# LarsDoorenbos/ccdm-stochastic-segmentation

Measured on AMD Instinct MI355X. Metric: segmentation samples/sec, LIDC 128x128 T=250, higher is better.
Workload: dtype f32 (conv products as split fp16 hi/lo x3 on MFMA, fp32 accumulate)

## Files before the change

ccdm_stochastic_segmentation_amd/csrc/ccdm_engine.hip:

```cpp
#include "ccdm_common.h"

#include <map>
#include <vector>

namespace ccdm {

__global__ void k_step_set(int32_t* p, int32_t v) { *p = v; }
__global__ void k_step_inc(int32_t* p) { *p += 1; }
__global__ void k_run_set(ccdm_post_run* dst, const ccdm_post_run v) { *dst = v; }
__global__ __launch_bounds__(256) void k_absmax(const float* __restrict__ x, size_t n4, float* out) {
    float m = 0.f;
    bool bad = false;
    for (size_t i = (size_t)blockIdx.x * blockDim.x + threadIdx.x; i < n4; i += (size_t)gridDim.x * blockDim.x) {
        const float4 v = reinterpret_cast<const float4*>(x)[i];
        bad |= !(fabsf(v.x) <= 3.0e38f) | !(fabsf(v.y) <= 3.0e38f) | !(fabsf(v.z) <= 3.0e38f) | !(fabsf(v.w) <= 3.0e38f);
        m = fmaxf(m, fmaxf(fmaxf(fabsf(v.x), fabsf(v.y)), fmaxf(fabsf(v.z), fabsf(v.w))));
    }
    if (bad) m = __builtin_inff();
#pragma unroll
    for (int off = 32; off > 0; off >>= 1) m = fmaxf(m, __shfl_xor(m, off));
    if ((threadIdx.x & 63) == 0) atomicMax(reinterpret_cast<unsigned*>(out), __float_as_uint(m));
}

struct Op {
    int kind;
    ccdm_conv_args conv;
    const float* qkv; float* out; int N, T, C, heads, order;
    const double* fin; double* fout; int S_in, S_out;
    ccdm_attn_block_args ab;
    ccdm_resample_args rs;
    ccdm_stem_args st;
    ccdm_head_args hd;
};

static int launch_op(const Op& op, hipStream_t s) {
    switch (op.kind) {
        case 6: return fail("engine: the head + epilogue op is launched with the epilogue's arguments");
        case 0: return launch_conv(op.conv, s);
        case 1: return launch_attention(op.qkv, op.out, op.N, op.T, op.T, op.C, op.heads, op.order, s);
        case 2: return launch_stats_fold(op.fin, op.N, op.S_in, op.C, op.S_out, op.fout, s);
        case 3: return launch_attn_block(op.ab, s);
        case 4: return launch_resample(op.rs, s);
        default: return launch_stem(op.st, s);
    }
}

}

struct ccdm_engine {
    int32_t* step = nullptr;
    std::vector<ccdm::Op> ops;
    ccdm_post_args post{};
    bool has_post = false;
    ccdm_post_run run{};
    ccdm_post_run* run_dev = nullptr;
    bool run_dirty = false;
    int next_row = 0;
    hipGraph_t graph = nullptr;
    hipGraphExec_t exec = nullptr;
    bool graph_valid = false;
    int graph_with_epilogue = -1;
    int captures = 0;
    struct Tap { std::vector<hipEvent_t> ev; int n = 0; };
    std::map<int, Tap> taps;
};

using namespace ccdm;

static void drop_graph(ccdm_engine* e) {
    if (e->exec) { (void)hipGraphExecDestroy(e->exec); e->exec = nullptr; }
    if (e->graph) { (void)hipGraphDestroy(e->graph); e->graph = nullptr; }
    e->graph_valid = false;
}

static int launch_step(ccdm_engine* e, int with_epilogue, hipStream_t s, bool profile) {
    for (size_t i = 0; i < e->ops.size(); ++i) {
        const Op& op = e->ops[i];
        ccdm_engine::Tap* tp = nullptr;
        if (profile) {
            auto it = e->taps.find((int)i);
            if (it != e->taps.end() && (size_t)(2 * it->second.n + 1) < it->second.ev.size()) tp = &it->second;
        }
        if (tp) (void)hipEventRecord(tp->ev[2 * tp->n], s);
        int rc;
        if (op.kind == 6) {
            rc = (with_epilogue && e->has_post) ? launch_head(op.hd, e->post, s) : fail("engine_run: this step ends in a fused head + epilogue op: with_epilogue must be 1 and an epilogue set");
        } else rc = launch_op(op, s);
        if (tp) { (void)hipEventRecord(tp->ev[2 * tp->n + 1], s); tp->n++; }
        if (rc) return rc;
    }
    if (with_epilogue && e->has_post && !(e->ops.size() && e->ops.back().kind == 6)) {
        int rc = launch_posterior(e->post, s);
        if (rc) return rc;
    }
    hipLaunchKernelGGL(k_step_inc, dim3(1), dim3(1), 0, s, e->step);
    CCDM_CHECK_LAUNCH("step_inc");
    return 0;
}

extern "C" ccdm_engine* ccdm_engine_create(int32_t* step_counter) {
    if (!step_counter) { fail("engine_create: null step counter"); return nullptr; }
    ccdm_engine* e = new ccdm_engine();
    e->step = step_counter;
    return e;
}

extern "C" void ccdm_engine_destroy(ccdm_engine* e) {
    if (!e) return;
    drop_graph(e);
    for (auto& kv : e->taps)
        for (hipEvent_t ev : kv.second.ev) (void)hipEventDestroy(ev);
    delete e;
}

extern "C" int ccdm_engine_add_conv(ccdm_engine* e, const ccdm_conv_args* a) {
    CCDM_REQUIRE(e && a, "engine_add_conv: null");
    Op op{};
    op.kind = 0;
    op.conv = *a;
    op.conv.step_ptr = e->step;
    e->ops.push_back(op);
    drop_graph(e);
    return (int)e->ops.size() - 1;
}

extern "C" int ccdm_engine_add_attention(ccdm_engine* e, const float* qkv, float* out, int N, int T, int C, int heads, int order) {
    CCDM_REQUIRE(e && qkv && out, "engine_add_attention: null");
    Op op{};
    op.kind = 1;
// ... 38 lines not shown
    CCDM_REQUIRE(e && a, "engine_add_stem: null");
    CCDM_REQUIRE(ccdm_stem_conv_supported(a->Cs, a->Cout, a->H, a->W, CCDM_PREC_F16X3), "engine_add_stem: Cs=%d Cout=%d %dx%d is not built", a->Cs, a->Cout, a->H, a->W);
    Op op{};
    op.kind = 5;
    op.st = *a;
    e->ops.push_back(op);
    drop_graph(e);
    return (int)e->ops.size() - 1;
}

extern "C" int ccdm_engine_add_head_posterior(ccdm_engine* e, const ccdm_head_args* a) {
    CCDM_REQUIRE(e && a, "engine_add_head_posterior: null");
    CCDM_REQUIRE(ccdm_head_posterior_supported(a->C, a->K, a->H, a->W, CCDM_PREC_F16X3), "engine_add_head_posterior: C=%d K=%d %dx%d is not built", a->C, a->K, a->H, a->W);
    Op op{};
    op.kind = 6;
    op.hd = *a;
    e->ops.push_back(op);
    drop_graph(e);
    return (int)e->ops.size() - 1;
}

extern "C" int ccdm_engine_set_epilogue(ccdm_engine* e, const ccdm_post_args* a) {
    CCDM_REQUIRE(e && a, "engine_set_epilogue: null");
    e->post = *a;
    e->post.step_ptr = e->step;
    e->has_post = true;
    if (e->run_dev) {
        e->post.run = e->run_dev;
        const ccdm_post_args& p = e->post;
        e->run = ccdm_post_run{p.noise, p.noise_step_stride, p.philox_seed, p.sample_offset, p.noise_row0, p.out_probs, p.out_onehot, p.posterior_out};
        e->run_dirty = true;
    }
    drop_graph(e);
    return 0;
}

extern "C" int ccdm_engine_num_ops(const ccdm_engine* e) { return e ? (int)e->ops.size() : -1; }
extern "C" int ccdm_engine_num_captures(const ccdm_engine* e) { return e ? e->captures : -1; }

extern "C" int ccdm_engine_set_run_block(ccdm_engine* e, void* dev_block) {
    CCDM_REQUIRE(e && e->has_post, "engine_set_run_block: no epilogue set");
    CCDM_REQUIRE(dev_block && (reinterpret_cast<uintptr_t>(dev_block) & 7) == 0, "engine_set_run_block: null or misaligned block");
    e->run_dev = static_cast<ccdm_post_run*>(dev_block);
    e->post.run = e->run_dev;
    const ccdm_post_args& p = e->post;
    e->run = ccdm_post_run{p.noise, p.noise_step_stride, p.philox_seed, p.sample_offset, p.noise_row0, p.out_probs, p.out_onehot, p.posterior_out};
    e->run_dirty = true;
    drop_graph(e);
    return 0;
}

extern "C" int ccdm_engine_set_run(ccdm_engine* e, const float* noise, int64_t noise_step_stride, int32_t noise_row0, uint64_t philox_seed,
                                   uint32_t sample_offset, float* out_probs, int64_t* out_onehot, float* posterior_out) {
    CCDM_REQUIRE(e && e->has_post, "engine_set_run: no epilogue set");
    if (e->run_dev) {
        const ccdm_post_run r{noise, noise_step_stride, philox_seed, sample_offset, noise_row0, out_probs, out_onehot, posterior_out};
        const ccdm_post_run& o = e->run;
        const bool same = o.noise == r.noise && o.noise_step_stride == r.noise_step_stride && o.philox_seed == r.philox_seed &&
                          o.sample_offset == r.sample_offset && o.noise_row0 == r.noise_row0 && o.out_probs == r.out_probs &&
                          o.out_onehot == r.out_onehot && o.posterior_out == r.posterior_out;
        if (!same) { e->run = r; e->run_dirty = true; }
        return 0;
    }
    ccdm_post_args& p = e->post;
    const bool same = p.noise == noise && p.noise_step_stride == noise_step_stride && p.noise_row0 == noise_row0 && p.philox_seed == philox_seed &&
                      p.sample_offset == sample_offset && p.out_probs == out_probs && p.out_onehot == out_onehot &&
                      p.posterior_out == posterior_out;
    if (!same) drop_graph(e);
    p.noise = noise; p.noise_step_stride = noise_step_stride; p.noise_row0 = noise_row0; p.philox_seed = philox_seed; p.sample_offset = sample_offset;
    p.out_probs = out_probs; p.out_onehot = out_onehot; p.posterior_out = posterior_out;
    return 0;
}

extern "C" int ccdm_engine_run(ccdm_engine* e, int first_row, int n_steps, int with_epilogue, int use_graph, void* stream) {
    CCDM_REQUIRE(e, "engine_run: null engine");
    CCDM_REQUIRE(n_steps >= 0, "engine_run: n_steps=%d", n_steps);
    hipStream_t s = (hipStream_t)stream;
    hipLaunchKernelGGL(k_step_set, dim3(1), dim3(1), 0, s, e->step, (int32_t)first_row);
    CCDM_CHECK_LAUNCH("step_set");
    e->next_row = first_row + n_steps;
    if (e->run_dev && e->run_dirty) {
        hipLaunchKernelGGL(k_run_set, dim3(1), dim3(1), 0, s, e->run_dev, e->run);
        CCDM_CHECK_LAUNCH("run_set");
        e->run_dirty = false;
    }
    const bool profile = !e->taps.empty();
    if (profile) {
        use_graph = 0;
        if (first_row == 0) for (auto& kv : e->taps) kv.second.n = 0;
    }
    if (use_graph) {
        if (!e->graph_valid || e->graph_with_epilogue != with_epilogue) {
            drop_graph(e);
            hipError_t err = hipStreamBeginCapture(s, hipStreamCaptureModeRelaxed);
            if (err != hipSuccess) return fail("engine_run: BeginCapture: %s", hipGetErrorString(err));
            const int rc = launch_step(e, with_epilogue, s, false);
            err = hipStreamEndCapture(s, &e->graph);
            if (rc) { if (e->graph) { (void)hipGraphDestroy(e->graph); e->graph = nullptr; } return rc; }
            if (err != hipSuccess) return fail("engine_run: EndCapture: %s", hipGetErrorString(err));
            err = hipGraphInstantiate(&e->exec, e->graph, nullptr, nullptr, 0);
            if (err != hipSuccess) return fail("engine_run: GraphInstantiate: %s", hipGetErrorString(err));
            e->graph_valid = true;
            e->graph_with_epilogue = with_epilogue;
            e->captures++;
        }
        for (int i = 0; i < n_steps; ++i) {
            hipError_t err = hipGraphLaunch(e->exec, s);
            if (err != hipSuccess) return fail("engine_run: GraphLaunch: %s", hipGetErrorString(err));
        }
        return 0;
    }
    for (int i = 0; i < n_steps; ++i) {
        int rc = launch_step(e, with_epilogue, s, profile);
        if (rc) return rc;
    }
    return 0;
}

extern "C" int ccdm_engine_profile_op(ccdm_engine* e, int op_index, int capacity) {
    CCDM_REQUIRE(e, "engine_profile_op: null engine");
    if (op_index < 0) {
        for (auto& kv : e->taps)
            for (hipEvent_t ev : kv.second.ev) (void)hipEventDestroy(ev);
        e->taps.clear();
        return 0;
    }
    CCDM_REQUIRE(op_index < (int)e->ops.size(), "engine_profile_op: op %d out of range", op_index);
    ccdm_engine::Tap& t = e->taps[op_index];
    t.n = 0;
    while ((int)t.ev.size() < 2 * capacity) {
        hipEvent_t ev;
        if (hipEventCreate(&ev) != hipSuccess) return fail("engine_profile_op: hipEventCreate failed");
        t.ev.push_back(ev);
    }
    return 0;
}

extern "C" int ccdm_engine_profile_read(ccdm_engine* e, int op_index, double* mean_ms, double* min_ms, double* max_ms) {
    CCDM_REQUIRE(e, "engine_profile_read: null engine");
    auto it = e->taps.find(op_index);
    CCDM_REQUIRE(it != e->taps.end(), "engine_profile_read: op %d is not tapped", op_index);
    ccdm_engine::Tap& t = it->second;
    double sum = 0, mn = 1e30, mx = 0;
    int n = 0;
    for (int i = 0; i < t.n; ++i) {
        float ms = 0.f;
// ... 67 lines not shown
```

ccdm_stochastic_segmentation_amd/engine.py:

```python
from __future__ import annotations

import ctypes as C
import math
from dataclasses import dataclass
from typing import Dict, List, Optional, Sequence, Tuple

import numpy as np
import torch

from . import hip
from .unet_spec import GN_EPS, UNetSpec


@dataclass
class DevTensor:
    buf: torch.Tensor
    C: int
    h: int
    w: int
    stats: Optional[torch.Tensor] = None
    slices: int = 0

    @property
    def ptr(self) -> int:
# ... 268 lines not shown
    def _layers(self, layers, src: Sequence[DevTensor]) -> DevTensor:
        h: Optional[DevTensor] = None
        for l in layers:
            cur = src if h is None else [h]
            if l.kind == "conv":
                if (cur[0] is self.xin and len(cur) == 1 and self.prec == hip.PREC_F16X3 and l.name not in self.f32_layers and not self.fine_slices
                        and self.lib.ccdm_stem_conv_supported(self.Cs, l.cout, self.H, self.W, hip.PREC_F16X3)):
                    h = self._stem(l.name, l.cout)
                else:
                    h = self._conv(cur, l.name, l.cout, 3)
            elif l.kind == "res":
                h = self._res(l.name, l, cur)
            elif l.kind == "attn":
                h = self._attn(l.name, l, cur[0])
            elif l.kind == "down":
                h = self._conv(cur, l.name + ".op", l.cout, 3, stride=2)
            elif l.kind == "up":
                h = self._conv(cur, l.name + ".conv", l.cout, 3, up=True)
            else:
                raise AssertionError(l.kind)
        return h

    def _build(self) -> None:
        spec, sd, N, H, W, K = self.spec, self._sd, self.N, self.H, self.W, self.K
        lib = self.lib
        missing = [k for k in spec.param_shapes() if k not in sd]
        if missing:
            raise KeyError(f"state_dict is missing {len(missing)} keys, e.g. {missing[:3]}")
        self.step = self._dev((1,), torch.int32, zero=True)
        self.rowmap = self._dev((N,), torch.int32, zero=True)
        self._handle = lib.ccdm_engine_create(self.step.data_ptr())
        if not self._handle:
            raise hip.CcdmHipError("engine_create: " + hip.last_error())
        self.op_names: List[str] = []
        self.op_info: List[dict] = []
        self.stem_onehot_on_load = False

        ted, mc = spec.time_embed_dim, spec.model_channels
        self.emb_offsets: Dict[str, int] = {}
        ws, bs, off = [], [], 0
        for name, l in spec.all_layers():
            if l.kind == "res":
                self.emb_offsets[name] = off
                ws.append(sd[name + ".emb_layers.1.weight"].numpy())
                bs.append(sd[name + ".emb_layers.1.bias"].numpy())
                off += ws[-1].shape[0]
        self.E = off
        self.wcat = self._upload(np.concatenate(ws, 0))
        self.bcat = self._upload(np.concatenate(bs, 0))
        self.te = [self._upload(sd[k].numpy()) for k in
                   ("time_embed.0.weight", "time_embed.0.bias", "time_embed.2.weight", "time_embed.2.bias")]
        S = self.max_steps
        self.sinus = self._dev((S, mc))
        self.emb_table = self._dev((S, self.E))
        self.step_table = self._dev((S, 4), zero=True)

        self.Cs = (K + self.C_img + 3) // 4 * 4
        self.xt = self._dev((N, H * W), torch.uint8, zero=True)
        self.xin = DevTensor(self._dev((N, H, W, self.Cs), zero=True), self.Cs, H, W)
        self.feat: Optional[DevTensor] = None
        if spec.feature_condition_idx:
            if self.feature_shape is None:
                raise ValueError("this model concatenates feature conditioning; feature_shape=(C,h,w) is required")
            fc, fh, fw = self.feature_shape
            if fc != spec.feature_channels:
                raise ValueError(f"feature_condition has {fc} channels, model expects {spec.feature_channels}")
# ... 59 lines not shown
        post.noise, post.noise_step_stride = 0, 0
        post.philox_seed, post.sample_offset = 0, 0
        post.xt_next = self.xt.data_ptr()
        post.xin, post.xin_stride = (0 if self.stem_onehot_on_load else self.xin.ptr), self.Cs
        post.out_probs, post.out_onehot, post.posterior_out = self.out_probs.data_ptr(), self.out_onehot.data_ptr(), 0
        self.flag = self._dev((1,), torch.int32, zero=True)
        post.noise_row0, post.range_flag = 0, self.flag.data_ptr()
        self._post = post
        hip.check(lib.ccdm_engine_set_epilogue(self._handle, C.byref(post)), "engine_set_epilogue")
        self.run_block = self._dev((hip.POST_RUN_BYTES // 8,), torch.int64, zero=True)
        hip.check(lib.ccdm_engine_set_run_block(self._handle, self.run_block.data_ptr()), "engine_set_run_block")
        self._sd = None
        self._tables_key = None
        self._per_sample_rows = False

    def __del__(self):
        try:
            if self._handle:
                self.lib.ccdm_engine_destroy(self._handle)
                self._handle = None
        except Exception:
            pass

    def _stream(self) -> int:
        return self.stream.cuda_stream

    def enter(self):
        self.stream.wait_stream(torch.cuda.current_stream(self.device))
        return torch.cuda.stream(self.stream)

    def leave(self) -> None:
        torch.cuda.current_stream(self.device).wait_stream(self.stream)

    def graph_captures(self) -> int:
        return int(self.lib.ccdm_engine_num_captures(self._handle))

    def describe_ops(self) -> List[str]:
        out = []
        buf = C.create_string_buffer(256)
        for i in range(self.n_unet_ops):
            self.lib.ccdm_engine_describe_op(self._handle, i, buf, 256)
            out.append(f"{i:3d} {self.op_names[i]}: {buf.value.decode()}")
        return out

    def set_inputs(self, xt_idx: torch.Tensor, cond: torch.Tensor, feat: Optional[torch.Tensor] = None) -> None:
        lib, s, N, HW = self.lib, self._stream(), self.N, self.H * self.W
        assert tuple(xt_idx.shape) == (N, self.H, self.W) and xt_idx.dtype == torch.uint8 and xt_idx.is_cuda
        assert tuple(cond.shape) == (N, self.C_img, self.H, self.W), (tuple(cond.shape), (N, self.C_img, self.H, self.W))
        cond = cond.to(self.device, torch.float32).contiguous()
        self.xt.copy_(xt_idx.reshape(N, HW))
        hip.check(lib.ccdm_nchw_to_nhwc(cond.data_ptr(), self.xin.ptr, N, self.C_img, HW, self.Cs, self.K, s), "nchw_to_nhwc")
        hip.check(lib.ccdm_onehot_to_xin(self.xt.data_ptr(), self.xin.ptr, N, HW, self.K, self.Cs, s), "onehot_to_xin")
        if self.feat is not None:
            if feat is None:
                raise ValueError("feature_condition is required by this model")
            f = self.feat
            assert tuple(feat.shape) == (N, f.C, f.h, f.w), tuple(feat.shape)
            feat = feat.to(self.device, torch.float32).contiguous()
            hip.check(lib.ccdm_nchw_to_nhwc(feat.data_ptr(), f.ptr, N, f.C, f.h * f.w, f.C, 0, s), "nchw_to_nhwc(feat)")
            hip.check(lib.ccdm_gn_stats(f.ptr, N, f.h * f.w, f.C, 1, f.stats_ptr, s), "gn_stats(feat)")
        self._cond_keepalive = (cond, feat)

    def set_tables(self, t_rows: Sequence[float], coeffs: Sequence[Tuple[float, float, int]], per_sample: bool = False) -> None:
        S = len(t_rows)
        if S > self.max_steps:
            raise ValueError(f"{S} table rows > max_steps {self.max_steps}")
# ... 131 lines not shown
```

ccdm_stochastic_segmentation_amd/hip.py:

```python
from __future__ import annotations

import ctypes as C
import os
import subprocess
from typing import Optional

_HERE = os.path.dirname(os.path.abspath(__file__))
ROOT = os.path.dirname(_HERE)
LIB_PATH = os.environ.get("CCDM_LIB") or os.path.join(_HERE, "libccdm_hip.so")
CSRC = os.path.join(_HERE, "csrc")
SOURCES = ["ccdm_conv.hip", "ccdm_conv_ks.hip", "ccdm_upconv.hip", "ccdm_stem.hip", "ccdm_head.hip", "ccdm_conv1x1.hip", "ccdm_misc.hip", "ccdm_attention.hip", "ccdm_attn_block.hip", "ccdm_sampler.hip", "ccdm_known.hip", "ccdm_guided.hip", "ccdm_metrics.hip", "ccdm_range.hip", "ccdm_resample.hip", "ccdm_engine.hip", "ccdm_vote.hip", "ccdm_segeval.hip", "ccdm_segexport.hip", "ccdm_csscore.hip", "ccdm_segcalib.hip", "ccdm_segboundary.hip", "ccdm_contourf.hip", "ccdm_uncscore.hip", "ccdm_lidcscore.hip", "ccdm_surfdist.hip", "ccdm_lesions.hip", "ccdm_lesionmatch.hip"]
HIPCC_FLAGS = ["--offload-arch=gfx950", "-O3", "-std=c++17", "-ffp-contract=off", "-mllvm", "-amdgpu-mfma-vgpr-form=1", "-fPIC", "-shared"]

ACT_NONE, ACT_SILU = 0, 1
RESAMPLE_AVGPOOL2, RESAMPLE_NEAREST_UP2 = 0, 1
ATTENTION_FORCE_VALU = 256
ATTENTION_VALU_WIDTHS = (4, 8, 12, 16, 24, 32, 48, 64)
DIAG_GENERAL_KERNEL = 2048 << 8
PREC_F32, PREC_F16X3 = 0, 1
PREC_F16 = 2
STEP_SAMPLE, STEP_LAST_CONFIDENCE, STEP_LAST_MAJORITY, STEP_LAST_KEEP, STEP_SOFTMAX_ONLY = 0, 1, 2, 3, 4
STATS_MAX_SLICES = 64
F16X3_LIMIT = 4094.0
STATS_FOLD_SLICES = 16
ABI_VERSION = 11
MAX_CLASSES = 255
CSSCORE_MAX_LABELS = 64
POST_DIAG_MANY = 256


class ConvArgs(C.Structure):
    _fields_ = [
        ("in0", C.c_void_p), ("in1", C.c_void_p), ("C0", C.c_int32), ("C1", C.c_int32),
        ("stats0", C.c_void_p), ("stats1", C.c_void_p), ("slices0", C.c_int32), ("slices1", C.c_int32),
        ("gamma", C.c_void_p), ("beta", C.c_void_p),
        ("eps", C.c_float), ("act", C.c_int32),
        ("film", C.c_int32), ("film_off", C.c_int32),
        ("N", C.c_int32), ("Hin", C.c_int32), ("Win", C.c_int32), ("Hout", C.c_int32), ("Wout", C.c_int32),
        ("ksize", C.c_int32), ("stride", C.c_int32), ("up", C.c_int32),
        ("w", C.c_void_p), ("bias", C.c_void_p), ("Cout", C.c_int32), ("prec", C.c_int32),
        ("emb_table", C.c_void_p), ("emb_stride", C.c_int32), ("emb_off", C.c_int32),
        ("emb_row_of_sample", C.c_void_p),
        ("step_ptr", C.c_void_p),
        ("resid", C.c_void_p),
        ("out", C.c_void_p),
        ("out_stats", C.c_void_p), ("out_slices", C.c_int32),
        ("skip0", C.c_void_p), ("skip1", C.c_void_p), ("SC0", C.c_int32), ("SC1", C.c_int32),
        ("skip_w", C.c_void_p),
        ("fine_slices", C.c_int32),
    ]


class PostArgs(C.Structure):
    _fields_ = [
        ("head", C.c_void_p), ("softmax", C.c_int32), ("head_stride", C.c_int32),
        ("xt", C.c_void_p),
        ("N", C.c_int32), ("HW", C.c_int32), ("K", C.c_int32),
        ("step_table", C.c_void_p), ("step_ptr", C.c_void_p),
# ... 122 lines not shown
                                 C.c_void_p, C.c_void_p, C.c_void_p, C.c_void_p, C.c_void_p, C.c_void_p]),
    "ccdm_csscore": (C.c_int, [C.c_void_p, C.c_int64, C.c_void_p, C.c_int, C.c_int, C.c_int, C.c_int, C.c_int, C.c_int, C.c_void_p, C.c_void_p,
                               C.c_void_p, C.c_int, C.c_void_p, C.c_void_p, C.c_void_p, C.c_int, C.c_int, C.c_void_p, C.c_void_p, C.c_void_p,
                               C.c_void_p, C.c_void_p]),
    "ccdm_csscore_ids": (C.c_int, [C.c_void_p, C.c_int, C.c_int, C.c_int, C.c_void_p, C.c_void_p, C.c_int, C.c_void_p, C.c_void_p, C.c_void_p,
                                   C.c_int, C.c_int, C.c_void_p, C.c_void_p, C.c_void_p, C.c_void_p, C.c_void_p]),
    "ccdm_segcalib_workspace_bytes": (C.c_size_t, [C.c_int, C.c_int, C.c_int, C.c_int, C.c_int]),
    "ccdm_segcalib": (C.c_int, [C.c_void_p, C.c_int64, C.c_void_p, C.c_void_p, C.c_int, C.c_int, C.c_int, C.c_int, C.c_int, C.c_int, C.c_int,
                                C.c_void_p, C.c_void_p, C.c_void_p, C.c_void_p, C.c_size_t, C.c_void_p]),
    "ccdm_segboundary_workspace_bytes": (C.c_size_t, [C.c_int, C.c_int, C.c_int]),
    "ccdm_segboundary": (C.c_int, [C.c_void_p, C.c_void_p, C.c_int, C.c_int, C.c_int, C.c_int, C.c_int, C.c_void_p, C.c_void_p, C.c_void_p,
                                   C.c_size_t, C.c_void_p]),
    "ccdm_contourf_workspace_bytes": (C.c_size_t, [C.c_int, C.c_int, C.c_int]),
    "ccdm_contourf": (C.c_int, [C.c_void_p, C.c_void_p, C.c_int, C.c_int, C.c_int, C.c_int, C.c_int, C.c_void_p, C.c_void_p, C.c_size_t,
                                C.c_void_p]),
    "ccdm_uncscore_workspace_bytes": (C.c_size_t, [C.c_int, C.c_int, C.c_int, C.c_int, C.c_int, C.c_int]),
    "ccdm_uncscore": (C.c_int, [C.c_void_p, C.c_int64, C.c_void_p, C.c_void_p, C.c_void_p, C.c_void_p, C.c_int, C.c_int, C.c_int, C.c_int,
                                C.c_int, C.c_int, C.c_int, C.c_int, C.c_int, C.c_void_p, C.c_void_p, C.c_void_p, C.c_size_t, C.c_void_p]),
    "ccdm_attention_ex": (C.c_int, [C.c_void_p, C.c_void_p, C.c_int, C.c_int, C.c_int, C.c_int, C.c_int, C.c_int, C.c_void_p]),
    "ccdm_layernorm": (C.c_int, [C.c_void_p, C.c_void_p, C.c_void_p, C.c_float, C.c_long, C.c_int, C.c_void_p, C.c_void_p]),
    "ccdm_gelu": (C.c_int, [C.c_void_p, C.c_size_t, C.c_void_p, C.c_void_p]),
    "ccdm_vit_key_resize": (C.c_int, [C.c_void_p, C.c_int, C.c_int, C.c_int, C.c_int, C.c_int, C.c_int, C.c_int, C.c_int, C.c_void_p,
                                      C.c_void_p]),
    "ccdm_mix_uniform": (C.c_int, [C.c_void_p, C.c_void_p, C.c_int, C.c_int, C.c_int, C.c_void_p, C.c_void_p]),
    "ccdm_theta_post": (C.c_int, [C.c_void_p, C.c_void_p, C.c_void_p, C.c_void_p, C.c_int, C.c_int, C.c_int, C.c_int, C.c_void_p, C.c_void_p]),
    "ccdm_kl_clamped": (C.c_int, [C.c_void_p, C.c_void_p, C.c_size_t, C.c_float, C.c_void_p, C.c_void_p]),
    "ccdm_nchw_to_nhwc": (C.c_int, [C.c_void_p, C.c_void_p, C.c_int, C.c_int, C.c_int, C.c_int, C.c_int, C.c_void_p]),
    "ccdm_onehot_to_xin": (C.c_int, [C.c_void_p, C.c_void_p, C.c_int, C.c_int, C.c_int, C.c_int, C.c_void_p]),
    "ccdm_engine_create": (C.c_void_p, [C.c_void_p]),
    "ccdm_engine_destroy": (None, [C.c_void_p]),
    "ccdm_engine_add_conv": (C.c_int, [C.c_void_p, C.POINTER(ConvArgs)]),
    "ccdm_engine_add_attention": (C.c_int, [C.c_void_p, C.c_void_p, C.c_void_p, C.c_int, C.c_int, C.c_int, C.c_int, C.c_int]),
    "ccdm_engine_set_epilogue": (C.c_int, [C.c_void_p, C.POINTER(PostArgs)]),
    "ccdm_engine_num_ops": (C.c_int, [C.c_void_p]),
    "ccdm_engine_num_captures": (C.c_int, [C.c_void_p]),
    "ccdm_engine_set_run_block": (C.c_int, [C.c_void_p, C.c_void_p]),
    "ccdm_engine_set_run": (C.c_int, [C.c_void_p, C.c_void_p, C.c_int64, C.c_int32, C.c_uint64, C.c_uint32, C.c_void_p, C.c_void_p, C.c_void_p]),
    "ccdm_engine_run": (C.c_int, [C.c_void_p, C.c_int, C.c_int, C.c_int, C.c_int, C.c_void_p]),
    "ccdm_engine_profile_op": (C.c_int, [C.c_void_p, C.c_int, C.c_int]),
    "ccdm_engine_profile_read": (C.c_int, [C.c_void_p, C.c_int, C.POINTER(C.c_double), C.POINTER(C.c_double), C.POINTER(C.c_double)]),
    "ccdm_engine_describe_op": (C.c_int, [C.c_void_p, C.c_int, C.c_char_p, C.c_int]),
}

_lib: Optional[C.CDLL] = None


class CcdmHipError(RuntimeError):
    pass


class CcdmRangeError(CcdmHipError):
    """The network output of a run was not finite: with PREC_F16X3 the signature of a staged activation beyond the fp16
    split's range (|a| >= 4094, include/ccdm_hip.h).  Outputs of that run are invalid."""


def build(force: bool = False, verbose: bool = False) -> str:
    from concurrent.futures import ThreadPoolExecutor
    srcs = [os.path.join(CSRC, s) for s in SOURCES]
    hdrs = [os.path.join(CSRC, h) for h in sorted(os.listdir(CSRC)) if h.endswith(".h")] + [os.path.join(ROOT, "include", "ccdm_hip.h")]
    objdir = os.path.join(_HERE, "build", "obj")
    os.makedirs(objdir, exist_ok=True)
    wanted = {os.path.basename(s) + ".o" for s in srcs}
    for f in os.listdir(objdir):
        if f.endswith(".o") and f not in wanted:
            os.remove(os.path.join(objdir, f))
    newest_hdr = max(os.path.getmtime(h) for h in hdrs)
# ... 137 lines not shown
```

ccdm_stochastic_segmentation_amd/models.py:

```python
from __future__ import annotations

import dataclasses
import logging
import math
from typing import Any, Callable, Dict, List, Optional, Sequence, Tuple, Union, cast

import numpy as np
import torch
from torch import Tensor, nn

from . import hip
from .engine import SamplerEngine
from .unet_spec import UNetSpec, make_unet_spec

LOGGER = logging.getLogger(__name__)

__all__ = ["build_model", "DiffusionModel", "DenoisingModel", "UNetModel", "OneHotCategoricalBCHW",
           "linear_schedule", "cosine_schedule", "step_values", "resample_walk", "pass_key"]


def linear_schedule(time_steps: int, start=1e-2, end=0.2) -> Tuple[Tensor, Tensor, Tensor]:
    betas = torch.linspace(start, end, time_steps)
    alphas = 1 - betas
    return betas, alphas, torch.cumprod(alphas, dim=0)
# ... 232 lines not shown
        self._weights_version += 1
        return r

    def forward(self, *args, **kwargs):
        raise RuntimeError("UNetModel has no eager forward; call it through DenoisingModel (HIP engine)")


HOST_NOISE_BLOCK_BYTES = 256 << 20


def auto_substreams(N: int, H: int, W: int) -> int:
    return 2 if (N >= 2 and N * H * W >= 32 * 128 * 128) else 1


class DenoisingModel(nn.Module):

    VIEW_FLIPS = {"hflip": 1, "vflip": 2, "hvflip": 3}

    KNOWN_FREE = 255

    def __init__(self, diffusion: DiffusionModel, unet: UNetModel, dataset_file: str, step_T_sample: str = "majority"):
        super().__init__()
        self.diffusion = diffusion
        self.unet = unet
        self.dataset_file = dataset_file
        self.step_T_sample = step_T_sample
        self.rng = "philox"
        self.philox_seed = 0
        self.philox_call = 0
        self.philox_advance = True
        self.sample_offset = 0
        self.noise_slice: Optional[Tuple[int, int]] = None
        self.use_graph = True
        self.substreams = 0
        self.calibrate_mode = True
        self.mode_choice: Dict[Any, dict] = {}
        self.last_mode: Optional[Tuple[int, bool]] = None
        self.prec = hip.PREC_F16X3
        self.on_range_error = "layers"
        self.f32_layers: set = set()
        self._auto_pins: set = set()
        self._auto_f32_from: Optional[int] = None
        self._auto_weights_key: Optional[Tuple[int, int]] = None
        self.range_events = {"overflows": 0, "layers_pinned": 0, "switched_to_f32": 0, "reset_on_new_weights": 0}
        self._range_probe: Optional[Dict[str, float]] = None
        self.slicing = "throughput"
        self._engines: Dict[Any, Tuple[int, SamplerEngine]] = {}

    @property
    def time_steps(self) -> int:
        return self.diffusion.time_steps

    def _fine_slices(self, N: int) -> int:
        if self.slicing not in ("throughput", "latency"):
            raise ValueError(f"slicing: {self.slicing!r} (expected 'throughput' or 'latency')")
        return 0 if self.slicing != "latency" else (2 if N <= 8 else 1)

    def forward(self, x: Tensor, condition: Tensor, feature_condition: Tensor = None, t: Optional[Tensor] = None,
                label_ref_logits: Optional[Tensor] = None, validation: bool = False, *,
                known_labels: Optional[Tensor] = None, resample: Optional[Tuple[int, int]] = None,
                evidence: Optional[Tensor] = None, temperature: Optional[float] = None,
                truncation: Optional[float] = None, views: Optional[Sequence[str]] = None) -> Union[Tensor, dict]:
        if evidence is not None and (self.training or validation):
            self._check_evidence(evidence, None, sampling=False)
        if self.training or validation:
            self._check_shaping(temperature, truncation, sampling=False)
# ... 5 lines not shown
        if self.training:
            if not isinstance(t, Tensor):
                raise ValueError("'t' needs to be a Tensor at training time")
            if not isinstance(x, Tensor):
                raise ValueError("'x' needs to be a Tensor at training time")
            return self.forward_step(x, condition, feature_condition, t)
        if validation:
            return self.forward_step(x, condition, feature_condition, t)
        if t is None:
            return self.forward_denoising(x, condition, feature_condition, label_ref_logits=label_ref_logits, known_labels=known_labels,
                                          resample=resample, evidence=evidence, temperature=temperature, truncation=truncation,
                                          views=views)
        return self.forward_denoising(x, condition, feature_condition, cast(int, t.item()), label_ref_logits, known_labels=known_labels,
                                      resample=resample, evidence=evidence, temperature=temperature, truncation=truncation, views=views)

    def _weights_key(self) -> Tuple[int, int]:
        return self.unet._weights_version, sum(int(p._version) for p in self.unet.parameters())

    def _engine(self, x: Tensor, condition: Tensor, feature_condition: Optional[Tensor], slot: int = 0) -> SamplerEngine:
        N, K, H, W = x.shape
        spec = self.unet.spec
        if feature_condition is not None and spec.feature_condition_unwired:
            raise RuntimeError(f"feature_condition given, but input block(s) {spec.feature_condition_unwired} were not widened for it "
                               "(feature_cond_encoder target_layer / output_stride do not line up): channel mismatch")
        fshape = tuple(feature_condition.shape[1:]) if feature_condition is not None else None
        if not spec.feature_condition_idx:
            fshape = None
        dev = next(self.unet.parameters()).device
        f32_layers = frozenset(self.f32_layers) if self.prec == hip.PREC_F16X3 else frozenset()
        key = (N, H, W, int(condition.shape[1]), fshape, str(dev), self.prec, slot, self._fine_slices(N), f32_layers)
        wkey = self._weights_key()
        hit = self._engines.get(key)
        if hit is not None and hit[0] == wkey:
            return hit[1]
        eng = SamplerEngine(spec, self.unet.state_dict(), N, H, W, K, int(condition.shape[1]), dev,
                            max_steps=self.time_steps, feature_shape=fshape, prec=self.prec, fine_slices=self._fine_slices(N),
                            f32_layers=f32_layers)
        self._engines = {k: v for k, v in self._engines.items() if v[0] == wkey}
        self._engines[key] = (wkey, eng)
        return eng

    def _philox_key(self) -> int:
        if int(self.philox_call) == 0:
            return int(self.philox_seed) & 0xFFFFFFFFFFFFFFFF
        z = (int(self.philox_seed) + 0x9E3779B97F4A7C15 * int(self.philox_call)) & 0xFFFFFFFFFFFFFFFF
        z = ((z ^ (z >> 30)) * 0xBF58476D1CE4E5B9) & 0xFFFFFFFFFFFFFFFF
        z = ((z ^ (z >> 27)) * 0x94D049BB133111EB) & 0xFFFFFFFFFFFFFFFF
        return z ^ (z >> 31)

    @staticmethod
    def _to_index(x: Tensor, device) -> Tensor:
        return x.argmax(dim=1).to(device=device, dtype=torch.uint8).contiguous()

    RANGE_MARGIN = 0.5

    def _probe_ranges(self, engines) -> None:
        if self._range_probe is None:
            return
        for eng in engines:
            hit = self._range_probe.get(id(eng))
            if hit is None:
                hit = self._range_probe[id(eng)] = (eng, eng.probe_buffer())
            eng.probe_ranges(hit[1])

    def _collect_probe(self) -> Optional[Dict[str, float]]:
        if self._range_probe is None:
            return None
        out: Dict[str, float] = {}
        for eng, buf in self._range_probe.values():
            for name, v in eng.read_ranges(buf).items():
                out[name] = max(out.get(name, 0.0), v)
        return out
# ... 398 lines not shown
        def prepare(nsub_: int):
            bounds = [(N * j) // nsub_ for j in range(nsub_ + 1)]
            parts_ = []
            for j in range(nsub_):
                lo, hi = bounds[j], bounds[j + 1]
                if views is None:
                    xs, cs = x[lo:hi], condition[lo:hi]
                    fc = feature_condition[lo:hi] if feature_condition is not None else None
                else:
                    xs, cs, fc = mirrored(x[lo:hi]), mirrored(condition[lo:hi]), None
                    if feature_condition is not None and self.unet.spec.feature_condition_idx:
                        fc = feature_condition[:, lo:hi].flatten(0, 1)
                eng = self._engine(xs, cs, fc, slot=j)
                with eng.enter():
                    eng.set_inputs(self._to_index(xs, eng.device), cs.to(eng.device), fc)
                    eng.set_tables([float(t) for t in t_values], table)
                parts_.append((eng, lo, hi))
            return parts_

        def run_row(eng, lo: int, hi: int, row: int, kp: int, renoise, noise, noise_row0_: int, graph_: bool):
            off = self.sample_offset + lo
            if renoise is not None:
                eng.renoise(*renoise, row, philox_seed=kp, sample_offset=off)
            eng.run(1, first_row=row, noise=noise, noise_row0=noise_row0_, philox_seed=kp, sample_offset=off, use_graph=graph_)
            if stop_at_x0:
                eng.guided_step(None if evidence is None else evidence[lo:hi], shaping, views, *coeffs[row], row, philox_seed=kp, sample_offset=off)
            if known is not None:
                eng.clamp_known_labels(known[lo:hi], clamp_c[row], coeffs[row][2], row, philox_seed=kp, sample_offset=off)

        def run_steps(parts_, s0_: int, s1_: int, noises_, noise_row0_: int, graph_: bool):
            if len(parts_) == 1 and not guide:
                parts_[0][0].run(s1_ - s0_, first_row=s0_, noise=noises_[0], noise_row0=noise_row0_, philox_seed=key,
                                 sample_offset=self.sample_offset, use_graph=graph_)
                return
            for e in range(s0_, s1_):
                row, p, _ = walk[e]
                for j, (eng, lo, hi) in enumerate(parts_):
                    run_row(eng, lo, hi, row, pass_key(key, p), renoise_p.get(e), noises_[j], noise_row0_, graph_)

        nsub = int(self.substreams) if int(self.substreams) > 0 else auto_substreams(V * N, H, W)
        nsub = max(1, min(nsub, N))
        use_graph = bool(self.use_graph)
        if (int(self.substreams) <= 0 and self.calibrate_mode and not host_rng and self._range_probe is None and nsub > 1
                and S >= self.CALIBRATION_MIN_STEPS and not guide):
            nsub, use_graph = self._calibrate_mode(x, condition, feature_condition, prepare, run_steps, nsub, use_graph, S)
        self.last_mode = (nsub, use_graph)
        parts = prepare(nsub)
        if host_rng:
            per_step = gN * H * W * K * 4
            blk = max(1, HOST_NOISE_BLOCK_BYTES // max(per_step, 1))
            blocks = [(s0, min(s0 + blk, S)) for s0 in range(0, S, blk)]
        else:
            blocks = [(0, len(walk))]
        if self._range_probe is not None:
            blocks = [(s, s + 1) for s in range(len(walk))]
        for s0, s1 in blocks:
            noises: List[Optional[Tensor]] = [None] * nsub
            if host_rng:
                host = torch.empty((s1 - s0, gN, H * W * K), dtype=torch.float32)
                for j in range(s0, s1):
                    if t_values[j] > 1:
                        host[j - s0].view(-1).exponential_(1)
                for j, (eng, lo, hi) in enumerate(parts):
                    with torch.cuda.stream(eng.stream):
                        noises[j] = host[:, first + lo:first + hi].contiguous().to(eng.device)
            run_steps(parts, s0, s1, noises, s0, use_graph)
# ... 63 lines not shown
```

include/ccdm_hip.h:

```cpp
#ifndef CCDM_HIP_H
#define CCDM_HIP_H

#include <stddef.h>
#include <stdint.h>

#ifdef __cplusplus
extern "C" {
#endif

#define CCDM_ABI_VERSION 11
#define CCDM_MAX_CHANNELS 1024
#define CCDM_STATS_MAX_SLICES 64
#define CCDM_STATS_FOLD_SLICES 16

int ccdm_version(void);
const char* ccdm_last_error_string(void);

int ccdm_gn_stats(const float* x , int N, int HW, int C, int slices,
                  double* stats , void* stream);

enum { CCDM_ACT_NONE = 0, CCDM_ACT_SILU = 1 };
enum { CCDM_PREC_F32 = 0,
       CCDM_PREC_F16X3 = 1,
       CCDM_PREC_F16 = 2 };
// ... 219 lines not shown
size_t ccdm_uncscore_workspace_bytes(int B, int H, int W, int K, int U, int M);
int ccdm_uncscore(const float* probs , int64_t pixel_stride, const uint8_t* cls ,
                  const uint8_t* labels , const float* maps , const float* ranges ,
                  int B, int h, int w, int H, int W, int K, int U, int M, int P, int64_t* pix ,
                  int64_t* patch , void* workspace, size_t workspace_bytes, void* stream);

int ccdm_vote_accumulate(const uint8_t* cls , const float* probs , int64_t src_stride,
                         int B, int HW, int K, float w, float* total ,
                         int32_t* counts , float* ent_sum , void* stream);
int ccdm_vote_finalize(const float* total , const int32_t* counts ,
                       const float* ent_sum , int B, int HW, int K, int S,
                       float* mean , uint8_t* vote ,
                       float* entropy , float* mutual_info , void* stream);
int ccdm_vote_reduce_stack(const uint8_t* stack , int B, int S, int HW, int K,
                           int32_t* counts , float* mean ,
                           uint8_t* vote , float* entropy , void* stream);

int ccdm_mix_uniform(const float* x , const float* s, int N, int K, int HW, float* out, void* stream);
int ccdm_theta_post(const float* xt , const float* x0 , const float* a, const float* c,
                    int N, int K, int HW, int prob_mode, float* out , void* stream);
int ccdm_kl_clamped(const float* p, const float* q, size_t n, float floor, float* out, void* stream);

int ccdm_attention_ex(const float* qkv , float* out , int N, int T, int T_alloc, int C,
                      int heads, int order, void* stream);
int ccdm_layernorm(const float* x, const float* gamma, const float* beta, float eps, long rows, int C, float* out, void* stream);
int ccdm_gelu(const float* x, size_t n, float* out, void* stream);
int ccdm_vit_key_resize(const float* qkv , int N, int T_alloc, int h0, int w0, int dim, int heads, int Ht, int Wt,
                        float* out , void* stream);

int ccdm_nchw_to_nhwc(const float* src, float* dst, int N, int C, int HW, int dst_stride, int dst_off, void* stream);
int ccdm_onehot_to_xin(const uint8_t* idx, float* xin, int N, int HW, int K, int xin_stride, void* stream);

typedef struct ccdm_engine ccdm_engine;

ccdm_engine* ccdm_engine_create(int32_t* step_counter );
void ccdm_engine_destroy(ccdm_engine* e);
int ccdm_engine_add_conv(ccdm_engine* e, const ccdm_conv_args* a);
int ccdm_engine_add_attention(ccdm_engine* e, const float* qkv, float* out, int N, int T, int C, int heads, int order);
int ccdm_engine_add_norm_qkv_attention(ccdm_engine* e, const ccdm_attn_block_args* a);
int ccdm_engine_add_stats_fold(ccdm_engine* e, const double* in, int N, int S_in, int C, int S_out, double* out);
int ccdm_engine_add_resample(ccdm_engine* e, const ccdm_resample_args* a);
int ccdm_engine_add_stem(ccdm_engine* e, const ccdm_stem_args* a);
int ccdm_engine_add_head_posterior(ccdm_engine* e, const ccdm_head_args* a);
int ccdm_engine_set_epilogue(ccdm_engine* e, const ccdm_post_args* a);
int ccdm_engine_num_ops(const ccdm_engine* e);
int ccdm_engine_num_captures(const ccdm_engine* e);
int ccdm_engine_set_run_block(ccdm_engine* e, void* dev_block);
int ccdm_engine_set_run(ccdm_engine* e, const float* noise, int64_t noise_step_stride, int32_t noise_row0,
                        uint64_t philox_seed, uint32_t sample_offset,
                        float* out_probs, int64_t* out_onehot, float* posterior_out);
int ccdm_engine_run(ccdm_engine* e, int first_row, int n_steps, int with_epilogue, int use_graph, void* stream);
int ccdm_engine_profile_op(ccdm_engine* e, int op_index, int capacity);
int ccdm_engine_profile_read(ccdm_engine* e, int op_index, double* mean_ms, double* min_ms, double* max_ms);
int ccdm_engine_input_absmax(ccdm_engine* e, float* out, int row, void* stream);
int ccdm_engine_describe_op(const ccdm_engine* e, int i, char* buf, int buflen);

#ifdef __cplusplus
}
#endif
#endif
```

Measured before the change: 88.67.

## Capture multiple diffusion steps per graph with a per-step row array

Adds the ability to capture G denoising steps into one HIP graph. A k_step_rows kernel writes per-step row indices into a device array, so each captured step reads its own row pointer rather than relying on a shared incrementing counter. This is meant to cut per-step graph launch and host overhead. The default G is 1, so the default path still launches one graph per step. That path now runs an extra kernel writing rows in place of the old increment kernel.

Result: no change. 88.61 (-0.1%).

```diff
diff --git a/ccdm_stochastic_segmentation_amd/csrc/ccdm_engine.hip b/ccdm_stochastic_segmentation_amd/csrc/ccdm_engine.hip
--- a/ccdm_stochastic_segmentation_amd/csrc/ccdm_engine.hip
+++ b/ccdm_stochastic_segmentation_amd/csrc/ccdm_engine.hip
@@ -6,7 +6,12 @@
 namespace ccdm {
 
 __global__ void k_step_set(int32_t* p, int32_t v) { *p = v; }
-__global__ void k_step_inc(int32_t* p) { *p += 1; }
+__global__ void k_step_rows(int32_t* step, int32_t* rows, int set, int32_t first) {
+    const int32_t base = set ? first : *step;
+    __syncthreads();
+    rows[threadIdx.x] = base + (int32_t)threadIdx.x;
+    if (threadIdx.x == 0) *step = base + (int32_t)blockDim.x;
+}
 __global__ void k_run_set(ccdm_post_run* dst, const ccdm_post_run v) { *dst = v; }
 __global__ __launch_bounds__(256) void k_absmax(const float* __restrict__ x, size_t n4, float* out) {
     float m = 0.f;
@@ -33,10 +38,10 @@
     ccdm_head_args hd;
 };
 
-static int launch_op(const Op& op, hipStream_t s) {
+static int launch_op(const Op& op, const int32_t* row, hipStream_t s) {
     switch (op.kind) {
         case 6: return fail("engine: the head + epilogue op is launched with the epilogue's arguments");
-        case 0: return launch_conv(op.conv, s);
+        case 0: { ccdm_conv_args a = op.conv; a.step_ptr = row; return launch_conv(a, s); }
         case 1: return launch_attention(op.qkv, op.out, op.N, op.T, op.T, op.C, op.heads, op.order, s);
         case 2: return launch_stats_fold(op.fin, op.N, op.S_in, op.C, op.S_out, op.fout, s);
         case 3: return launch_attn_block(op.ab, s);
@@ -56,9 +61,10 @@
     ccdm_post_run* run_dev = nullptr;
     bool run_dirty = false;
     int next_row = 0;
-    hipGraph_t graph = nullptr;
-    hipGraphExec_t exec = nullptr;
-    bool graph_valid = false;
+    int32_t* rows = nullptr;
+    int graph_steps = 1;
+    struct Graph { hipGraph_t graph = nullptr; hipGraphExec_t exec = nullptr; int len = 0; };
+    Graph multi, single;
     int graph_with_epilogue = -1;
     int captures = 0;
     struct Tap { std::vector<hipEvent_t> ev; int n = 0; };
@@ -68,12 +74,22 @@
 using namespace ccdm;
 
 static void drop_graph(ccdm_engine* e) {
-    if (e->exec) { (void)hipGraphExecDestroy(e->exec); e->exec = nullptr; }
-    if (e->graph) { (void)hipGraphDestroy(e->graph); e->graph = nullptr; }
-    e->graph_valid = false;
-}
-
-static int launch_step(ccdm_engine* e, int with_epilogue, hipStream_t s, bool profile) {
+    for (ccdm_engine::Graph* g : {&e->multi, &e->single}) {
+        if (g->exec) { (void)hipGraphExecDestroy(g->exec); g->exec = nullptr; }
+        if (g->graph) { (void)hipGraphDestroy(g->graph); g->graph = nullptr; }
+        g->len = 0;
+    }
+}
+
+static int launch_rows(ccdm_engine* e, int n, int set, int first, hipStream_t s) {
+    hipLaunchKernelGGL(k_step_rows, dim3(1), dim3(n), 0, s, e->step, e->rows, set, (int32_t)first);
+    CCDM_CHECK_LAUNCH("step_rows");
+    return 0;
+}
+
+static int launch_step(ccdm_engine* e, int with_epilogue, const int32_t* row, hipStream_t s, bool profile) {
+    ccdm_post_args post = e->post;
+    post.step_ptr = row;
     for (size_t i = 0; i < e->ops.size(); ++i) {
         const Op& op = e->ops[i];
         ccdm_engine::Tap* tp = nullptr;
@@ -84,17 +100,34 @@
         if (tp) (void)hipEventRecord(tp->ev[2 * tp->n], s);
         int rc;
         if (op.kind == 6) {
-            rc = (with_epilogue && e->has_post) ? launch_head(op.hd, e->post, s) : fail("engine_run: this step ends in a fused head + epilogue op: with_epilogue must be 1 and an epilogue set");
-        } else rc = launch_op(op, s);
+            rc = (with_epilogue && e->has_post) ? launch_head(op.hd, post, s) : fail("engine_run: this step ends in a fused head + epilogue op: with_epilogue must be 1 and an epilogue set");
+        } else rc = launch_op(op, row, s);
         if (tp) { (void)hipEventRecord(tp->ev[2 * tp->n + 1], s); tp->n++; }
         if (rc) return rc;
     }
     if (with_epilogue && e->has_post && !(e->ops.size() && e->ops.back().kind == 6)) {
-        int rc = launch_posterior(e->post, s);
+        int rc = launch_posterior(post, s);
         if (rc) return rc;
     }
-    hipLaunchKernelGGL(k_step_inc, dim3(1), dim3(1), 0, s, e->step);
-    CCDM_CHECK_LAUNCH("step_inc");
+    return 0;
+}
+
+static int ensure_graph(ccdm_engine* e, ccdm_engine::Graph* g, int len, int with_epilogue, hipStream_t s) {
+    if (g->exec && g->len == len) return 0;
+    if (g->exec) { (void)hipGraphExecDestroy(g->exec); g->exec = nullptr; }
+    if (g->graph) { (void)hipGraphDestroy(g->graph); g->graph = nullptr; }
+    g->len = 0;
+    hipError_t err = hipStreamBeginCapture(s, hipStreamCaptureModeRelaxed);
+    if (err != hipSuccess) return fail("engine_run: BeginCapture: %s", hipGetErrorString(err));
+    int rc = launch_rows(e, len, 0, 0, s);
+    for (int j = 0; j < len && !rc; ++j) rc = launch_step(e, with_epilogue, e->rows + j, s, false);
+    err = hipStreamEndCapture(s, &g->graph);
+    if (rc) { if (g->graph) { (void)hipGraphDestroy(g->graph); g->graph = nullptr; } return rc; }
+    if (err != hipSuccess) return fail("engine_run: EndCapture: %s", hipGetErrorString(err));
+    err = hipGraphInstantiate(&g->exec, g->graph, nullptr, nullptr, 0);
+    if (err != hipSuccess) return fail("engine_run: GraphInstantiate: %s", hipGetErrorString(err));
+    g->len = len;
+    e->captures++;
     return 0;
 }
 
@@ -199,6 +232,15 @@
         e->run_dirty = true;
     }
     drop_graph(e);
+    return 0;
+}
+
+extern "C" int ccdm_engine_set_graph_steps(ccdm_engine* e, int G, int32_t* rows) {
+    CCDM_REQUIRE(e && rows, "engine_set_graph_steps: null");
+    CCDM_REQUIRE(G >= 1 && G <= CCDM_ENGINE_GRAPH_STEPS_MAX, "engine_set_graph_steps: G=%d (1..%d)", G, CCDM_ENGINE_GRAPH_STEPS_MAX);
+    if (G != e->graph_steps || rows != e->rows) drop_graph(e);
+    e->graph_steps = G;
+    e->rows = rows;
     return 0;
 }
 
@@ -242,9 +284,8 @@
 extern "C" int ccdm_engine_run(ccdm_engine* e, int first_row, int n_steps, int with_epilogue, int use_graph, void* stream) {
     CCDM_REQUIRE(e, "engine_run: null engine");
     CCDM_REQUIRE(n_steps >= 0, "engine_run: n_steps=%d", n_steps);
+    CCDM_REQUIRE(e->rows, "engine_run: no row array set (ccdm_engine_set_graph_steps)");
     hipStream_t s = (hipStream_t)stream;
-    hipLaunchKernelGGL(k_step_set, dim3(1), dim3(1), 0, s, e->step, (int32_t)first_row);
-    CCDM_CHECK_LAUNCH("step_set");
     e->next_row = first_row + n_steps;
     if (e->run_dev && e->run_dirty) {
         hipLaunchKernelGGL(k_run_set, dim3(1), dim3(1), 0, s, e->run_dev, e->run);
@@ -256,29 +297,31 @@
         use_graph = 0;
         if (first_row == 0) for (auto& kv : e->taps) kv.second.n = 0;
     }
+    if (use_graph || n_steps == 0) {
+        hipLaunchKernelGGL(k_step_set, dim3(1), dim3(1), 0, s, e->step, (int32_t)first_row);
+        CCDM_CHECK_LAUNCH("step_set");
+    }
     if (use_graph) {
-        if (!e->graph_valid || e->graph_with_epilogue != with_epilogue) {
-            drop_graph(e);
-            hipError_t err = hipStreamBeginCapture(s, hipStreamCaptureModeRelaxed);
-            if (err != hipSuccess) return fail("engine_run: BeginCapture: %s", hipGetErrorString(err));
-            const int rc = launch_step(e, with_epilogue, s, false);
-            err = hipStreamEndCapture(s, &e->graph);
-            if (rc) { if (e->graph) { (void)hipGraphDestroy(e->graph); e->graph = nullptr; } return rc; }
-            if (err != hipSuccess) return fail("engine_run: EndCapture: %s", hipGetErrorString(err));
-            err = hipGraphInstantiate(&e->exec, e->graph, nullptr, nullptr, 0);
-            if (err != hipSuccess) return fail("engine_run: GraphInstantiate: %s", hipGetErrorString(err));
-            e->graph_valid = true;
-            e->graph_with_epilogue = with_epilogue;
-            e->captures++;
-        }
-        for (int i = 0; i < n_steps; ++i) {
-            hipError_t err = hipGraphLaunch(e->exec, s);
-            if (err != hipSuccess) return fail("engine_run: GraphLaunch: %s", hipGetErrorString(err));
+        if (e->graph_with_epilogue != with_epilogue) drop_graph(e);
+        e->graph_with_epilogue = with_epilogue;
+        const int G = e->graph_steps;
+        const int full = G > 1 ? n_steps / G : 0;
+        for (int pass = 0; pass < 2; ++pass) {
+            ccdm_engine::Graph* g = pass ? &e->single : &e->multi;
+            const int reps = pass ? n_steps - full * G : full;
+            if (!reps) continue;
+            const int rc = ensure_graph(e, g, pass ? 1 : G, with_epilogue, s);
+            if (rc) return rc;
+            for (int i = 0; i < reps; ++i) {
+                hipError_t err = hipGraphLaunch(g->exec, s);
+                if (err != hipSuccess) return fail("engine_run: GraphLaunch: %s", hipGetErrorString(err));
+            }
         }
         return 0;
     }
     for (int i = 0; i < n_steps; ++i) {
-        int rc = launch_step(e, with_epilogue, s, profile);
+        int rc = launch_rows(e, 1, i == 0, first_row, s);
+        if (!rc) rc = launch_step(e, with_epilogue, e->rows, s, profile);
         if (rc) return rc;
     }
     return 0;
diff --git a/ccdm_stochastic_segmentation_amd/engine.py b/ccdm_stochastic_segmentation_amd/engine.py
--- a/ccdm_stochastic_segmentation_amd/engine.py
+++ b/ccdm_stochastic_segmentation_amd/engine.py
@@ -324,6 +324,9 @@
         self._handle = lib.ccdm_engine_create(self.step.data_ptr())
         if not self._handle:
             raise hip.CcdmHipError("engine_create: " + hip.last_error())
+        self.step_rows = self._dev((hip.GRAPH_STEPS_MAX,), torch.int32, zero=True)
+        self.graph_steps = 0
+        self.set_graph_steps(hip.GRAPH_STEPS_DEFAULT)
         self.op_names: List[str] = []
         self.op_info: List[dict] = []
         self.stem_onehot_on_load = False
@@ -449,6 +452,11 @@
     def leave(self) -> None:
         torch.cuda.current_stream(self.device).wait_stream(self.stream)
 
+    def set_graph_steps(self, G: int) -> None:
+        if int(G) != self.graph_steps:
+            hip.check(self.lib.ccdm_engine_set_graph_steps(self._handle, int(G), self.step_rows.data_ptr()), "engine_set_graph_steps")
+            self.graph_steps = int(G)
+
     def graph_captures(self) -> int:
         return int(self.lib.ccdm_engine_num_captures(self._handle))
 
diff --git a/ccdm_stochastic_segmentation_amd/hip.py b/ccdm_stochastic_segmentation_amd/hip.py
--- a/ccdm_stochastic_segmentation_amd/hip.py
+++ b/ccdm_stochastic_segmentation_amd/hip.py
@@ -24,6 +24,7 @@
 F16X3_LIMIT = 4094.0
 STATS_FOLD_SLICES = 16
 ABI_VERSION = 11
+GRAPH_STEPS_MAX, GRAPH_STEPS_DEFAULT = 32, 1
 MAX_CLASSES = 255
 CSSCORE_MAX_LABELS = 64
 POST_DIAG_MANY = 256
@@ -212,6 +213,7 @@
     "ccdm_engine_add_conv": (C.c_int, [C.c_void_p, C.POINTER(ConvArgs)]),
     "ccdm_engine_add_attention": (C.c_int, [C.c_void_p, C.c_void_p, C.c_void_p, C.c_int, C.c_int, C.c_int, C.c_int, C.c_int]),
     "ccdm_engine_set_epilogue": (C.c_int, [C.c_void_p, C.POINTER(PostArgs)]),
+    "ccdm_engine_set_graph_steps": (C.c_int, [C.c_void_p, C.c_int, C.c_void_p]),
     "ccdm_engine_num_ops": (C.c_int, [C.c_void_p]),
     "ccdm_engine_num_captures": (C.c_int, [C.c_void_p]),
     "ccdm_engine_set_run_block": (C.c_int, [C.c_void_p, C.c_void_p]),
diff --git a/ccdm_stochastic_segmentation_amd/models.py b/ccdm_stochastic_segmentation_amd/models.py
--- a/ccdm_stochastic_segmentation_amd/models.py
+++ b/ccdm_stochastic_segmentation_amd/models.py
@@ -288,6 +288,7 @@
         self.sample_offset = 0
         self.noise_slice: Optional[Tuple[int, int]] = None
         self.use_graph = True
+        self.graph_steps = hip.GRAPH_STEPS_DEFAULT
         self.substreams = 0
         self.calibrate_mode = True
         self.mode_choice: Dict[Any, dict] = {}
@@ -359,12 +360,14 @@
         wkey = self._weights_key()
         hit = self._engines.get(key)
         if hit is not None and hit[0] == wkey:
+            hit[1].set_graph_steps(self.graph_steps)
             return hit[1]
         eng = SamplerEngine(spec, self.unet.state_dict(), N, H, W, K, int(condition.shape[1]), dev,
                             max_steps=self.time_steps, feature_shape=fshape, prec=self.prec, fine_slices=self._fine_slices(N),
                             f32_layers=f32_layers)
         self._engines = {k: v for k, v in self._engines.items() if v[0] == wkey}
         self._engines[key] = (wkey, eng)
+        eng.set_graph_steps(self.graph_steps)
         return eng
 
     def _philox_key(self) -> int:
@@ -829,6 +832,13 @@
             if len(parts_) == 1 and not guide:
                 parts_[0][0].run(s1_ - s0_, first_row=s0_, noise=noises_[0], noise_row0=noise_row0_, philox_seed=key,
                                  sample_offset=self.sample_offset, use_graph=graph_)
+                return
+            if not guide and graph_ and int(self.graph_steps) > 1:
+                G = int(self.graph_steps)
+                for e in range(s0_, s1_, G):
+                    for j, (eng, lo, hi) in enumerate(parts_):
+                        eng.run(min(G, s1_ - e), first_row=e, noise=noises_[j], noise_row0=noise_row0_, philox_seed=key,
+                                sample_offset=self.sample_offset + lo, use_graph=True)
                 return
             for e in range(s0_, s1_):
                 row, p, _ = walk[e]
diff --git a/include/ccdm_hip.h b/include/ccdm_hip.h
--- a/include/ccdm_hip.h
+++ b/include/ccdm_hip.h
@@ -275,6 +275,8 @@
 int ccdm_onehot_to_xin(const uint8_t* idx, float* xin, int N, int HW, int K, int xin_stride, void* stream);
 
 typedef struct ccdm_engine ccdm_engine;
+#define CCDM_ENGINE_GRAPH_STEPS_MAX 32
+#define CCDM_ENGINE_GRAPH_STEPS_DEFAULT 1
 
 ccdm_engine* ccdm_engine_create(int32_t* step_counter );
 void ccdm_engine_destroy(ccdm_engine* e);
@@ -286,6 +288,7 @@
 int ccdm_engine_add_stem(ccdm_engine* e, const ccdm_stem_args* a);
 int ccdm_engine_add_head_posterior(ccdm_engine* e, const ccdm_head_args* a);
 int ccdm_engine_set_epilogue(ccdm_engine* e, const ccdm_post_args* a);
+int ccdm_engine_set_graph_steps(ccdm_engine* e, int G, int32_t* rows );
 int ccdm_engine_num_ops(const ccdm_engine* e);
 int ccdm_engine_num_captures(const ccdm_engine* e);
 int ccdm_engine_set_run_block(ccdm_engine* e, void* dev_block);
```
